# chrischoy/CUDA-FFT-Convolution

Hardware: AMD Instinct MI355X
Metric: Gpixel-filters/s (padded FFT size) (higher is better)
Workload: dtype f32; 1 GPU; cfg3: 4096x4096 image (F=1), 256 kernels of 127x127 in total -> 256 maps of 4224x4224 per step, filter-sharded; filters_total=256, filters_per_gpu=256, hip_graph_replay=False, clock_warm_steps=88, dynamic_tiles=1, parallelism=single GPU

## Files before the change

### cuda-fft-convolution_amd/csrc/butterflies.hpp

```cpp
#pragma once
#include <type_traits>
#include "dft_consts.hpp"
#include "fc_common.hpp"

#ifndef FC_DFT_PFA
#define FC_DFT_PFA 1
#endif

namespace fc {

template <int SGN>
FC_HD c32 mul_j(c32 a) {
    if constexpr (SGN > 0) return mk(-a.y, a.x);
    else return mk(a.y, -a.x);
}
template <int SGN>
FC_HD c32 add_j(c32 a, c32 b) {
    if constexpr (SGN > 0) return add_jb(a, b);
    else return sub_jb(a, b);
}
template <int SGN>
FC_HD c32 sub_j(c32 a, c32 b) {
    if constexpr (SGN > 0) return sub_jb(a, b);
    else return add_jb(a, b);
}

template <int R, int K, int SGN>
FC_HD c32 mul_root(c32 a) {
    constexpr int k = ((K % R) + R) % R;
    if constexpr (k == 0) {
        return a;
    } else if constexpr (2 * k == R) {
        return mk(-a.x, -a.y);
    } else if constexpr (4 * k == R) {
        return mul_j<SGN>(a);
    } else if constexpr (4 * k == 3 * R) {
        return mul_j<-SGN>(a);
    } else if constexpr ((8 * k) % R == 0) {
        constexpr int q = (8 * k) / R;
        constexpr float h = 0.70710678118654752f;
        constexpr float sc = (q == 1 || q == 7) ? 1.f : -1.f;
        constexpr float ss = ((q == 1 || q == 3) ? 1.f : -1.f) * (SGN > 0 ? 1.f : -1.f);
        c32 t = (ss * sc > 0.f) ? add_jb(a, a) : sub_jb(a, a);
        return scale(t, sc * h);
    } else {
        constexpr float c = Roots<R>::c[k];
        constexpr float s = (SGN > 0 ? 1.f : -1.f) * Roots<R>::s[k];
        return fma_js(s, a, scale(a, c));
    }
}

constexpr int smallest_factor(int r) {
    if (r % 4 == 0 && r > 4) return 4;
    if (r % 2 == 0) return 2;
    for (int f = 3; f * f <= r; f += 2)
        if (r % f == 0) return f;
    return r;
}
constexpr bool is_prime(int r) { return r >= 2 && smallest_factor(r) == r && r != 4; }

template <int R, int SGN, class Enable = void>
struct Dft;

template <int SGN>
struct Dft<1, SGN, void> {
    static FC_HD void run(c32 (&)[1]) {}
    template <int NZ>
    static FC_HD void run_nz(c32 (&)[1]) {}
};

template <int SGN>
struct Dft<2, SGN, void> {
    static FC_HD void run(c32 (&v)[2]) {
        c32 a = v[0], b = v[1];
        v[0] = a + b;
        v[1] = a - b;
    }
    template <int NZ>
    static FC_HD void run_nz(c32 (&v)[2]) {
        if constexpr (NZ <= 1) v[1] = v[0];
        else run(v);
    }
};

template <int SGN>
struct Dft<4, SGN, void> {
    static FC_HD void run(c32 (&v)[4]) {
        c32 s0 = v[0] + v[2], s1 = v[0] - v[2];
        c32 s2 = v[1] + v[3], d = v[1] - v[3];
        v[0] = s0 + s2;
        v[1] = add_j<SGN>(s1, d);
        v[2] = s0 - s2;
        v[3] = sub_j<SGN>(s1, d);
    }
    template <int NZ>
    static FC_HD void run_nz(c32 (&v)[4]) {
        if constexpr (NZ <= 1) {
            v[1] = v[0]; v[2] = v[0]; v[3] = v[0];
        } else if constexpr (NZ == 2) {
            const c32 a = v[0], b = v[1];
            v[0] = a + b;
            v[1] = add_j<SGN>(a, b);
            v[2] = a - b;
            v[3] = sub_j<SGN>(a, b);
        } else {
            run(v);
        }
    }
};

template <int P, int SGN>
struct DftOddPrime {
    static FC_HD void run(c32 (&v)[P]) {
        constexpr int H = (P - 1) / 2;
        c32 s[H], d[H];
        static_for<0, H>([&](auto k_) {
            constexpr int k = decltype(k_)::value;
            s[k] = v[k + 1] + v[P - 1 - k];
            d[k] = v[k + 1] - v[P - 1 - k];
        });
        c32 v0 = v[0];
        c32 x0 = v0;
        static_for<0, H>([&](auto k_) { x0 = x0 + s[decltype(k_)::value]; });
        v[0] = x0;
        static_for<1, H + 1>([&](auto m_) {
            constexpr int m = decltype(m_)::value;
            c32 A = v0, B = mk(0.f, 0.f);
            static_for<0, H>([&](auto k_) {
                constexpr int k = decltype(k_)::value;
                constexpr int idx = (m * (k + 1)) % P;
                constexpr float c = Roots<P>::c[idx];
                constexpr float sn = Roots<P>::s[idx];
                A = fma_real(c, s[k], A);
                if constexpr (k == 0) B = scale(d[k], sn);
                else B = fma_real(sn, d[k], B);
            });
            v[m] = add_j<SGN>(A, B);
            v[P - m] = sub_j<SGN>(A, B);
        });
    }
};

template <int R, int SGN>
struct Dft<R, SGN, std::enable_if_t<(R >= 3) && (R % 2 == 1) && is_prime(R)>> {
    static FC_HD void run(c32 (&v)[R]) { DftOddPrime<R, SGN>::run(v); }
    template <int NZ>
    static FC_HD void run_nz(c32 (&v)[R]) {
        if constexpr (NZ <= 1) static_for<1, R>([&](auto k_) { v[decltype(k_)::value] = v[0]; });
        else DftOddPrime<R, SGN>::run(v);
    }
};

template <int R1, int R2, int SGN>
struct DftCT {
    static constexpr int R = R1 * R2;
    static FC_HD void run(c32 (&v)[R]) {
        c32 y[R];
        static_for<0, R2>([&](auto b_) {
            constexpr int b = decltype(b_)::value;
            c32 t[R1];
            static_for<0, R1>([&](auto a_) {
                constexpr int a = decltype(a_)::value;
                t[a] = v[a * R2 + b];
            });
            Dft<R1, SGN>::run(t);
            static_for<0, R1>([&](auto c_) {
                constexpr int c = decltype(c_)::value;
                y[c * R2 + b] = mul_root<R, b * c, SGN>(t[c]);
            });
        });
        static_for<0, R1>([&](auto c_) {
            constexpr int c = decltype(c_)::value;
            c32 t[R2];
            static_for<0, R2>([&](auto b_) {
                constexpr int b = decltype(b_)::value;
                t[b] = y[c * R2 + b];
            });
            Dft<R2, SGN>::run(t);
            static_for<0, R2>([&](auto k_) {
                constexpr int k = decltype(k_)::value;
                v[c + R1 * k] = t[k];
            });
        });
    }
};

template <int R1, int R2, int SGN, int NZ>
struct DftCTnz {
    static constexpr int R = R1 * R2;
    static_assert(NZ >= 1 && NZ <= R2, "pruned composite: the non-zero inputs must lie in the first sub-block");
    static FC_HD void run(c32 (&v)[R]) {
        c32 y[R];
        static_for<0, NZ>([&](auto b_) {
            constexpr int b = decltype(b_)::value;
            const c32 x = v[b];
            static_for<0, R1>([&](auto c_) {
                constexpr int c = decltype(c_)::value;
                y[c * R2 + b] = mul_root<R, b * c, SGN>(x);
            });
        });
        static_for<0, R1>([&](auto c_) {
            constexpr int c = decltype(c_)::value;
            c32 t[R2];
            static_for<0, R2>([&](auto b_) {
                constexpr int b = decltype(b_)::value;
                if constexpr (b < NZ) t[b] = y[c * R2 + b];
                else t[b] = mk(0.f, 0.f);
            });
            Dft<R2, SGN>::template run_nz<NZ>(t);
            static_for<0, R2>([&](auto k_) {
                constexpr int k = decltype(k_)::value;
                v[c + R1 * k] = t[k];
            });
        });
    }
};

template <int A, int B, int SGN>
struct DftPFA {
    static constexpr int R = A * B;
    static constexpr int in_idx(int a, int b) {
        int n = 0;
        while (n % A != a || n % B != b) ++n;
        return n;
    }
    static constexpr int out_idx(int ka, int kb) { return (ka * B + kb * A) % R; }

    static FC_HD void run(c32 (&v)[R]) {
        c32 y[R];
        static_for<0, B>([&](auto b_) {
            constexpr int b = decltype(b_)::value;
            c32 t[A];
            static_for<0, A>([&](auto a_) {
                constexpr int a = decltype(a_)::value, n = in_idx(a, b);
                t[a] = v[n];
            });
            Dft<A, SGN>::run(t);
            static_for<0, A>([&](auto k_) {
                constexpr int k = decltype(k_)::value;
                y[k * B + b] = t[k];
            });
        });
        second_stage<B>(v, y);
    }

    template <int NZ>
    static FC_HD void run_nz(c32 (&v)[R]) {
        static_assert(NZ >= 1 && NZ <= B, "pruned prime-factor form: the non-zero inputs must lie in [0, B)");
        c32 y[R];
        static_for<0, NZ>([&](auto b_) {
            constexpr int b = decltype(b_)::value;
            const c32 x = v[b];
            static_for<0, A>([&](auto k_) {
                constexpr int k = decltype(k_)::value;
                y[k * B + b] = mul_root<A, (b % A) * k, SGN>(x);
            });
        });
        second_stage<NZ>(v, y);
    }

  private:
    template <int NZ>
    static FC_HD void second_stage(c32 (&v)[R], const c32 (&y)[R]) {
        static_for<0, A>([&](auto ka_) {
            constexpr int ka = decltype(ka_)::value;
            c32 t[B];
            static_for<0, B>([&](auto b_) {
                constexpr int b = decltype(b_)::value;
                if constexpr (b < NZ) t[b] = y[ka * B + b];
                else t[b] = mk(0.f, 0.f);
            });
            if constexpr (NZ < B) Dft<B, SGN>::template run_nz<NZ>(t);
            else Dft<B, SGN>::run(t);
            static_for<0, B>([&](auto kb_) {
                constexpr int kb = decltype(kb_)::value, k = out_idx(ka, kb);
                v[k] = t[kb];
            });
        });
    }
};

constexpr int gcd_c(int a, int b) { return b == 0 ? a : gcd_c(b, a % b); }
constexpr int pfa_first(int r) {
    int p = 2;
    while (r % p != 0) ++p;
    int q = 1;
    while (r % (q * p) == 0) q *= p;
    return q == r ? 0 : (q < r / q ? q : r / q);
}

template <int R, int SGN>
struct Dft<R, SGN, std::enable_if_t<(R > 4) && !is_prime(R)>> {
    static constexpr int F1 = smallest_factor(R), F2 = R / smallest_factor(R);
    static constexpr int PA = FC_DFT_PFA ? pfa_first(R) : 0, PB = PA ? R / PA : 0;
    static_assert(PA == 0 || gcd_c(PA, PB) == 1, "prime-factor split needs coprime factors");
    static FC_HD void run(c32 (&v)[R]) {
        if constexpr (PA > 0) DftPFA<PA, PB, SGN>::run(v);
        else DftCT<F1, F2, SGN>::run(v);
    }
    template <int NZ>
    static FC_HD void run_nz(c32 (&v)[R]) {
        if constexpr (PA > 0 && NZ >= 1 && NZ <= PB) DftPFA<PA, PB, SGN>::template run_nz<NZ>(v);
        else if constexpr (NZ >= 1 && NZ <= F2) DftCTnz<F1, F2, SGN, NZ>::run(v);
        else run(v);
    }
};

}
```

Measured before the change: 388.7 Gpixel-filters/s.

## Fold twiddle multiplies into butterfly add/sub and prune zero inputs in composite DFTs

Adds an addsub_root helper that merges twiddle rotations by trivial roots (1, -1, ±j, and optionally eighth roots) into the butterfly add/sub, and a rotated radix-4 kernel that takes the twiddle inside. Composite Cooley-Tukey DFTs gain a generalized zero-pruned path with per-column non-zero counts, used by default through a FOLD template parameter. Some sizes (16, 32, inverse 8, inverse 24) are excluded by heuristic. The goal is fewer FLOPs and registers in the register-resident FFT butterflies, at the cost of different instruction schedules and register pressure that could hurt occupancy.

New measurement: 389.9 Gpixel-filters/s (median of 6 runs). Within noise of the previous version (+0.3%).

```diff
diff --git a/cuda-fft-convolution_amd/csrc/butterflies.hpp b/cuda-fft-convolution_amd/csrc/butterflies.hpp
--- a/cuda-fft-convolution_amd/csrc/butterflies.hpp
+++ b/cuda-fft-convolution_amd/csrc/butterflies.hpp
@@ -5,6 +5,9 @@
 
 #ifndef FC_DFT_PFA
 #define FC_DFT_PFA 1
+#endif
+#ifndef FC_DFT_FOLD
+#define FC_DFT_FOLD 1
 #endif
 
 namespace fc {
@@ -50,6 +53,36 @@
     }
 }
 
+template <int R, int K, int SGN, int FOLD>
+FC_HD void addsub_root(c32 a, c32 t, c32& sum, c32& diff) {
+    constexpr int k = ((K % R) + R) % R;
+    if constexpr (FOLD >= 1 && k == 0) {
+        sum = a + t;
+        diff = a - t;
+    } else if constexpr (FOLD >= 1 && 2 * k == R) {
+        sum = a - t;
+        diff = a + t;
+    } else if constexpr (FOLD >= 1 && 4 * k == R) {
+        sum = add_j<SGN>(a, t);
+        diff = sub_j<SGN>(a, t);
+    } else if constexpr (FOLD >= 1 && 4 * k == 3 * R) {
+        sum = sub_j<SGN>(a, t);
+        diff = add_j<SGN>(a, t);
+    } else if constexpr (FOLD >= 2 && (8 * k) % R == 0) {
+        constexpr int q = (8 * k) / R;
+        constexpr float h = 0.70710678118654752f;
+        constexpr float sc = (q == 1 || q == 7) ? 1.f : -1.f;
+        constexpr float ss = ((q == 1 || q == 3) ? 1.f : -1.f) * (SGN > 0 ? 1.f : -1.f);
+        const c32 u = (ss * sc > 0.f) ? add_jb(t, t) : sub_jb(t, t);
+        sum = fma_real(sc * h, u, a);
+        diff = fma_real(-sc * h, u, a);
+    } else {
+        const c32 y = mul_root<R, K, SGN>(t);
+        sum = a + y;
+        diff = a - y;
+    }
+}
+
 constexpr int smallest_factor(int r) {
     if (r % 4 == 0 && r > 4) return 4;
     if (r % 2 == 0) return 2;
@@ -59,18 +92,26 @@
 }
 constexpr bool is_prime(int r) { return r >= 2 && smallest_factor(r) == r && r != 4; }
 
-template <int R, int SGN, class Enable = void>
+constexpr int dft_fold(int r, int sgn) {
+    return (r == 16 || r == 32 || (r == 8 && sgn > 0)) ? 0 : FC_DFT_FOLD;
+}
+
+constexpr int dft_fold_run(int r, int sgn, int fold) {
+    return (r == 24 && sgn < 0) ? 0 : fold;
+}
+
+template <int R, int SGN, int FOLD = dft_fold(R, SGN), class Enable = void>
 struct Dft;
 
-template <int SGN>
-struct Dft<1, SGN, void> {
+template <int SGN, int FOLD>
+struct Dft<1, SGN, FOLD, void> {
     static FC_HD void run(c32 (&)[1]) {}
     template <int NZ>
     static FC_HD void run_nz(c32 (&)[1]) {}
 };
 
-template <int SGN>
-struct Dft<2, SGN, void> {
+template <int SGN, int FOLD>
+struct Dft<2, SGN, FOLD, void> {
     static FC_HD void run(c32 (&v)[2]) {
         c32 a = v[0], b = v[1];
         v[0] = a + b;
@@ -83,8 +124,8 @@
     }
 };
 
-template <int SGN>
-struct Dft<4, SGN, void> {
+template <int SGN, int FOLD>
+struct Dft<4, SGN, FOLD, void> {
     static FC_HD void run(c32 (&v)[4]) {
         c32 s0 = v[0] + v[2], s1 = v[0] - v[2];
         c32 s2 = v[1] + v[3], d = v[1] - v[3];
@@ -103,8 +144,38 @@
             v[1] = add_j<SGN>(a, b);
             v[2] = a - b;
             v[3] = sub_j<SGN>(a, b);
+        } else if constexpr (NZ == 3 && FOLD >= 1) {
+            const c32 s0 = v[0] + v[2], s1 = v[0] - v[2], b = v[1];
+            v[0] = s0 + b;
+            v[1] = add_j<SGN>(s1, b);
+            v[2] = s0 - b;
+            v[3] = sub_j<SGN>(s1, b);
         } else {
             run(v);
+        }
+    }
+    template <int NZ, int R, int C>
+    static FC_HD void run_rot(c32 (&v)[4]) {
+        if constexpr (NZ <= 1) {
+            v[1] = v[0]; v[2] = v[0]; v[3] = v[0];
+        } else if constexpr (NZ == 2) {
+            v[1] = mul_root<R, C, SGN>(v[1]);
+            run_nz<2>(v);
+        } else {
+            c32 s0, s1, s2, d;
+            addsub_root<R, 2 * C, SGN, FOLD>(v[0], v[2], s0, s1);
+            const c32 y1 = mul_root<R, C, SGN>(v[1]);
+            if constexpr (NZ >= 4) {
+                addsub_root<R, 3 * C, SGN, FOLD>(y1, v[3], s2, d);
+            } else if constexpr (FOLD >= 1) {
+                s2 = y1; d = y1;
+            } else {
+                s2 = y1 + v[3]; d = y1 - v[3];
+            }
+            v[0] = s0 + s2;
+            v[1] = add_j<SGN>(s1, d);
+            v[2] = s0 - s2;
+            v[3] = sub_j<SGN>(s1, d);
         }
     }
 };
@@ -141,8 +212,8 @@
     }
 };
 
-template <int R, int SGN>
-struct Dft<R, SGN, std::enable_if_t<(R >= 3) && (R % 2 == 1) && is_prime(R)>> {
+template <int R, int SGN, int FOLD>
+struct Dft<R, SGN, FOLD, std::enable_if_t<(R >= 3) && (R % 2 == 1) && is_prime(R)>> {
     static FC_HD void run(c32 (&v)[R]) { DftOddPrime<R, SGN>::run(v); }
     template <int NZ>
     static FC_HD void run_nz(c32 (&v)[R]) {
@@ -151,10 +222,15 @@
     }
 };
 
-template <int R1, int R2, int SGN>
+template <int R1, int R2, int SGN, int FOLD>
 struct DftCT {
     static constexpr int R = R1 * R2;
+    static constexpr int nz1(int nz, int b) { return b < nz ? (nz - b + R2 - 1) / R2 : 0; }
     static FC_HD void run(c32 (&v)[R]) {
+        if constexpr (FOLD == 0) run_unfolded(v);
+        else run_nz<R>(v);
+    }
+    static FC_HD void run_unfolded(c32 (&v)[R]) {
         c32 y[R];
         static_for<0, R2>([&](auto b_) {
             constexpr int b = decltype(b_)::value;
@@ -163,7 +239,7 @@
                 constexpr int a = decltype(a_)::value;
                 t[a] = v[a * R2 + b];
             });
-            Dft<R1, SGN>::run(t);
+            Dft<R1, SGN, 0>::run(t);
             static_for<0, R1>([&](auto c_) {
                 constexpr int c = decltype(c_)::value;
                 y[c * R2 + b] = mul_root<R, b * c, SGN>(t[c]);
@@ -176,11 +252,58 @@
                 constexpr int b = decltype(b_)::value;
                 t[b] = y[c * R2 + b];
             });
-            Dft<R2, SGN>::run(t);
+            Dft<R2, SGN, 0>::run(t);
             static_for<0, R2>([&](auto k_) {
                 constexpr int k = decltype(k_)::value;
                 v[c + R1 * k] = t[k];
             });
+        });
+    }
+    template <int NZ>
+    static FC_HD void run_nz(c32 (&v)[R]) {
+        static_assert(NZ >= 1 && NZ <= R, "pruned composite: NZ counts the leading non-zero inputs");
+        constexpr int NZ2 = NZ < R2 ? NZ : R2;
+        c32 y[R];
+        static_for<0, NZ2>([&](auto b_) {
+            constexpr int b = decltype(b_)::value, n = nz1(NZ, b);
+            c32 t[R1];
+            static_for<0, R1>([&](auto a_) {
+                constexpr int a = decltype(a_)::value;
+                if constexpr (a < n) t[a] = v[a * R2 + b];
+                else t[a] = mk(0.f, 0.f);
+            });
+            if constexpr (n < R1) Dft<R1, SGN, FOLD>::template run_nz<n>(t);
+            else Dft<R1, SGN, FOLD>::run(t);
+            static_for<0, R1>([&](auto c_) {
+                constexpr int c = decltype(c_)::value;
+                y[c * R2 + b] = t[c];
+            });
+        });
+        static_for<0, R1>([&](auto c_) {
+            constexpr int c = decltype(c_)::value;
+            if constexpr (R2 == 2) {
+                if constexpr (NZ2 == 1) {
+                    v[c] = y[c * 2];
+                    v[c + R1] = y[c * 2];
+                } else {
+                    addsub_root<R, c, SGN, FOLD>(y[c * 2], y[c * 2 + 1], v[c], v[c + R1]);
+                }
+            } else {
+                c32 t[R2];
+                static_for<0, R2>([&](auto b_) {
+                    constexpr int b = decltype(b_)::value;
+                    if constexpr (b >= NZ2) t[b] = mk(0.f, 0.f);
+                    else if constexpr (R2 == 4) t[b] = y[c * R2 + b];
+                    else t[b] = mul_root<R, b * c, SGN>(y[c * R2 + b]);
+                });
+                if constexpr (R2 == 4) Dft<4, SGN, FOLD>::template run_rot<NZ2, R, c>(t);
+                else if constexpr (NZ2 < R2) Dft<R2, SGN, FOLD>::template run_nz<NZ2>(t);
+                else Dft<R2, SGN, FOLD>::run(t);
+                static_for<0, R2>([&](auto k_) {
+                    constexpr int k = decltype(k_)::value;
+                    v[c + R1 * k] = t[k];
+                });
+            }
         });
     }
 };
@@ -207,7 +330,7 @@
                 if constexpr (b < NZ) t[b] = y[c * R2 + b];
                 else t[b] = mk(0.f, 0.f);
             });
-            Dft<R2, SGN>::template run_nz<NZ>(t);
+            Dft<R2, SGN, 0>::template run_nz<NZ>(t);
             static_for<0, R2>([&](auto k_) {
                 constexpr int k = decltype(k_)::value;
                 v[c + R1 * k] = t[k];
@@ -216,7 +339,7 @@
     }
 };
 
-template <int A, int B, int SGN>
+template <int A, int B, int SGN, int FOLD>
 struct DftPFA {
     static constexpr int R = A * B;
     static constexpr int in_idx(int a, int b) {
@@ -235,7 +358,7 @@
                 constexpr int a = decltype(a_)::value, n = in_idx(a, b);
                 t[a] = v[n];
             });
-            Dft<A, SGN>::run(t);
+            Dft<A, SGN, FOLD>::run(t);
             static_for<0, A>([&](auto k_) {
                 constexpr int k = decltype(k_)::value;
                 y[k * B + b] = t[k];
@@ -270,8 +393,8 @@
                 if constexpr (b < NZ) t[b] = y[ka * B + b];
                 else t[b] = mk(0.f, 0.f);
             });
-            if constexpr (NZ < B) Dft<B, SGN>::template run_nz<NZ>(t);
-            else Dft<B, SGN>::run(t);
+            if constexpr (NZ < B) Dft<B, SGN, FOLD>::template run_nz<NZ>(t);
+            else Dft<B, SGN, FOLD>::run(t);
             static_for<0, B>([&](auto kb_) {
                 constexpr int kb = decltype(kb_)::value, k = out_idx(ka, kb);
                 v[k] = t[kb];
@@ -289,19 +412,21 @@
     return q == r ? 0 : (q < r / q ? q : r / q);
 }
 
-template <int R, int SGN>
-struct Dft<R, SGN, std::enable_if_t<(R > 4) && !is_prime(R)>> {
+template <int R, int SGN, int FOLD>
+struct Dft<R, SGN, FOLD, std::enable_if_t<(R > 4) && !is_prime(R)>> {
     static constexpr int F1 = smallest_factor(R), F2 = R / smallest_factor(R);
     static constexpr int PA = FC_DFT_PFA ? pfa_first(R) : 0, PB = PA ? R / PA : 0;
     static_assert(PA == 0 || gcd_c(PA, PB) == 1, "prime-factor split needs coprime factors");
     static FC_HD void run(c32 (&v)[R]) {
-        if constexpr (PA > 0) DftPFA<PA, PB, SGN>::run(v);
-        else DftCT<F1, F2, SGN>::run(v);
+        constexpr int FR = dft_fold_run(R, SGN, FOLD);
+        if constexpr (PA > 0) DftPFA<PA, PB, SGN, FR>::run(v);
+        else DftCT<F1, F2, SGN, FR>::run(v);
     }
     template <int NZ>
     static FC_HD void run_nz(c32 (&v)[R]) {
-        if constexpr (PA > 0 && NZ >= 1 && NZ <= PB) DftPFA<PA, PB, SGN>::template run_nz<NZ>(v);
-        else if constexpr (NZ >= 1 && NZ <= F2) DftCTnz<F1, F2, SGN, NZ>::run(v);
+        if constexpr (PA > 0 && NZ >= 1 && NZ <= PB) DftPFA<PA, PB, SGN, FOLD>::template run_nz<NZ>(v);
+        else if constexpr (FOLD == 0 && NZ >= 1 && NZ <= F2) DftCTnz<F1, F2, SGN, NZ>::run(v);
+        else if constexpr (FOLD >= 1 && NZ >= 1 && (NZ <= F2 || (PA == 0 && NZ < R))) DftCT<F1, F2, SGN, FOLD>::template run_nz<NZ>(v);
         else run(v);
     }
 };
```
